# Hongyang-Du/VideoGPA

Measured on AMD Instinct MI355X. Metric: DPO preference-pair steps/sec, CogVideoX-5B 49f@480x720, higher is better.
Workload: dtype bf16; 1 GPU; BASELINE configs[1]: CogVideoX-5B T2V full (42 blocks, D=3072, 48x64 heads), 49f x 480x720 -> paired latents [1,2,13,16,60,90], S=17776 tokens, 42 blocks, LoRA r=64 on to_q/to_k/to_v/to_out.0, 1 pair/GPU/step, optimizer step every step; random-init weights; layers=42, pairs_per_gpu=1, parallelism=dp1

## Files before the change

include/videogpa_hip.h:

```cpp
#ifndef VIDEOGPA_HIP_H
#define VIDEOGPA_HIP_H

#include <stddef.h>
#include <stdint.h>

#ifdef __cplusplus
extern "C" {
#endif

typedef struct ihipStream_t* vgpa_stream_t;

#define VGPA_OK 0
#define VGPA_ERR_INVALID (-1)
#define VGPA_ERR_LAUNCH (-2)
#define VGPA_ERR_WORKSPACE (-3)

size_t vgpa_dpo_loss_workspace_bytes(int64_t B);
int32_t vgpa_dpo_loss_fwd(const void* v_win, const void* v_lose, const void* v_win_ref, const void* v_lose_ref,
                          const void* tgt_win, const void* tgt_lose, int64_t B, int64_t N, int64_t stride_pred,
                          int64_t stride_ref, int64_t stride_tgt, int32_t dtype, float beta, float label_smoothing,
                          int32_t loss_type, int32_t flags, float* out5, float* dlogit, float* errs, void* workspace,
                          size_t ws_bytes, vgpa_stream_t stream);
int32_t vgpa_dpo_loss_bwd(const void* v_win, const void* v_lose, const void* tgt_win, const void* tgt_lose, int64_t B,
                          int64_t N, int64_t stride_pred, int64_t stride_tgt, int64_t stride_grad, int32_t dtype, float beta,
// ... 37 lines not shown
                                int64_t text_len, void* dx, void* dy_q8, float* dy_scale, vgpa_stream_t stream);
int32_t vgpa_gate_residual(const void* x, const void* y, const float* gate_v, const float* gate_t, int64_t mod_stride,
                           int64_t B, int64_t S, int64_t D, int64_t text_len, void* out, vgpa_stream_t stream);
int32_t vgpa_gelu_tanh_fwd(const void* u, int64_t n, void* out, vgpa_stream_t stream);
int32_t vgpa_gelu_tanh_bwd(const void* u, const void* dy, int64_t n, void* du, vgpa_stream_t stream);

int32_t vgpa_qknorm_rope_fwd(const void* q_in, const void* k_in, void* q_out, void* k_out, const int64_t* qin_strides,
                             const int64_t* kin_strides, const int64_t* qout_strides, const int64_t* kout_strides,
                             const float* wq, const float* bq, const float* wk, const float* bk, const float* rope_cos,
                             const float* rope_sin, int64_t text_len, int64_t B, int64_t H, int64_t S, int64_t head_dim,
                             float eps, float q_out_scale, int32_t rope_mode, vgpa_stream_t stream);
int32_t vgpa_qknorm_rope_bwd(const void* dq_out, const void* dk_out, const void* q_in, const void* k_in, void* dq_in,
                             void* dk_in, const int64_t* dqout_strides, const int64_t* dkout_strides,
                             const int64_t* qin_strides, const int64_t* kin_strides, const int64_t* dqin_strides,
                             const int64_t* dkin_strides, const float* wq, const float* wk, const float* rope_cos,
                             const float* rope_sin, int64_t text_len, int64_t B, int64_t H, int64_t S, int64_t head_dim,
                             float eps, int32_t rope_mode, vgpa_stream_t stream);

int32_t vgpa_attn_bwd_delta_res(const void* o, const void* o_res, int32_t res_kind, const void* d_o, const int64_t* o_strides, const int64_t* ores_strides,
                                const int64_t* do_strides, float* delta, int64_t B, int64_t H, int64_t S, int64_t head_dim,
                                vgpa_stream_t stream);
size_t vgpa_attn_bwd_split_workspace_bytes(int64_t B, int64_t H, int64_t S);
int32_t vgpa_attn_bwd_dq_w1(const void* q, const void* k, const void* v, const void* d_o, const float* lse2, const float* delta,
                            void* dq, const int64_t* q_strides, const int64_t* k_strides, const int64_t* v_strides,
                            const int64_t* do_strides, const int64_t* dq_strides, int64_t B, int64_t H, int64_t S, int64_t head_dim,
                            float scale, int32_t split_mode, void* workspace, size_t ws_bytes, vgpa_stream_t stream);
size_t vgpa_attn_fwd_w1_workspace_bytes(int64_t B, int64_t H, int64_t S);
#define VGPA_RES_NONE 0
#define VGPA_RES_BF16 1
#define VGPA_RES_8 2
int32_t vgpa_attn_fwd_w1_res(const void* q, const void* k, const void* v, void* o, void* o_res, int32_t res_kind, float* lse2, const int64_t* q_strides,
                             const int64_t* k_strides, const int64_t* v_strides, const int64_t* o_strides, const int64_t* ores_strides,
                             int64_t B, int64_t H, int64_t S, int64_t head_dim, float scale, int32_t split_mode, void* workspace,
                             size_t ws_bytes, vgpa_stream_t stream);
int32_t vgpa_attn_fwd_online_res(const void* q, const void* k, const void* v, void* o, void* o_res, int32_t res_kind, float* lse2, const int64_t* q_strides,
                                 const int64_t* k_strides, const int64_t* v_strides, const int64_t* o_strides, const int64_t* ores_strides,
                                 int64_t B, int64_t H, int64_t S, int64_t head_dim, float scale, int32_t split_mode, void* workspace,
                                 size_t ws_bytes, vgpa_stream_t stream);
int32_t vgpa_attn_bwd_prep_w1_res(const void* o, const void* o_res, int32_t res_kind, const void* d_o, const float* lse2, const int64_t* o_strides,
                                  const int64_t* ores_strides, const int64_t* do_strides, float* delta, float* stats, int64_t B, int64_t H,
                                  int64_t S, int64_t head_dim, vgpa_stream_t stream);
int32_t vgpa_attn_bwd_dkv_w1(const void* q, const void* k, const void* v, const void* d_o, const float* stats, void* dk, void* dv,
                             const int64_t* q_strides, const int64_t* k_strides, const int64_t* v_strides, const int64_t* do_strides,
                             const int64_t* dk_strides, const int64_t* dv_strides, int64_t B, int64_t H, int64_t S, int64_t head_dim,
                             float scale, int32_t split_mode, void* workspace, size_t ws_bytes, vgpa_stream_t stream);

int32_t vgpa_lora_down(const void* X, int64_t ldx, const void* A, void* T, int64_t ldt, int64_t M, int64_t K, int64_t R,
                       vgpa_stream_t stream);
int32_t vgpa_lora_up_add(void* Y, int64_t ldy, const void* T, int64_t ldt, const void* Bw, int64_t ldb, float s, int64_t M,
                         int64_t N, int64_t rp, int32_t accumulate, vgpa_stream_t stream);
size_t vgpa_lora_grad_workspace_bytes(int64_t M, int64_t P, int64_t Q);
int32_t vgpa_lora_grad_ws(const void* U, int64_t ldu, const void* V, int64_t ldv, float* G, int64_t ldg, float s, int64_t M,
                          int64_t P, int64_t Q, void* workspace, size_t ws_bytes, vgpa_stream_t stream);
int32_t vgpa_lora_ext_refresh(const float* A, const float* B, float s, int64_t r, int64_t K, int64_t Dn, void* a_cat, void* wt_tail, int64_t ld_wt,
                              void* w_tail, int64_t ld_w, void* sbt, vgpa_stream_t stream);

#ifdef VGPA_VARIANTS
int32_t vgpa_gemm_bf16(const void* X, int64_t ldx, const void* W, int64_t ldw, const void* bias, void* C, int64_t ldc, void* aux,
                       int64_t ldaux, int32_t M, int32_t N, int32_t K, int32_t epilogue, vgpa_stream_t stream);
#endif

size_t vgpa_attn128_fwd_workspace_bytes(int64_t B, int64_t H, int64_t Sq);
int32_t vgpa_attn128_fwd(const void* q, const void* k, const void* v, void* o, float* lse2, const int64_t* q_strides, const int64_t* k_strides,
                         const int64_t* v_strides, const int64_t* o_strides, void* o_res8, const int64_t* ores_strides, int64_t B, int64_t H,
                         int64_t Sq, int64_t Skv, float scale, void* workspace, size_t ws_bytes, vgpa_stream_t stream);
size_t vgpa_attn128_fwd_f8_workspace_bytes(int64_t B, int64_t H, int64_t Sq, int64_t Skv);
int32_t vgpa_attn128_fwd_f8(const void* q, const void* k, const void* v, void* o, float* lse2, const int64_t* q_strides, const int64_t* k_strides,
                            const int64_t* v_strides, const int64_t* o_strides, void* o_res8, const int64_t* ores_strides, void* q_deq, void* k_deq,
                            void* v_deq, const int64_t* qd_strides, const int64_t* kd_strides, const int64_t* vd_strides, int64_t B, int64_t H,
                            int64_t Sq, int64_t Skv, float scale, void* workspace, size_t ws_bytes, vgpa_stream_t stream);
size_t vgpa_attn128_bwd_workspace_bytes(int64_t B, int64_t H, int64_t Sq);
int32_t vgpa_attn128_bwd(const void* q, const void* k, const void* v, const void* o, const void* d_o, const float* lse2, void* dq, void* dk,
                         void* dv, const int64_t* q_strides, const int64_t* k_strides, const int64_t* v_strides,
                         const int64_t* o_strides, const int64_t* do_strides, const int64_t* dq_strides, const int64_t* dk_strides,
                         const int64_t* dv_strides, const void* o_res8, const int64_t* ores_strides, int64_t B, int64_t H, int64_t Sq, int64_t Skv,
                         float scale, int32_t dkv_mode, void* workspace, size_t ws_bytes, vgpa_stream_t stream);
int32_t vgpa_attn128_bwd_prescaled(const void* q, const void* k, const void* v, const void* o, const void* d_o, const float* lse2, void* dq, void* dk,
                                   void* dv, const int64_t* q_strides, const int64_t* k_strides, const int64_t* v_strides,
                                   const int64_t* o_strides, const int64_t* do_strides, const int64_t* dq_strides, const int64_t* dk_strides,
                                   const int64_t* dv_strides, const void* o_res8, const int64_t* ores_strides, int64_t B, int64_t H, int64_t Sq, int64_t Skv,
                                   float scale, int32_t dkv_mode, void* workspace, size_t ws_bytes, vgpa_stream_t stream);

int32_t vgpa_wan_ln_mod_fwd(const void* x, int32_t x_dtype, const void* y, const float* gate, float* x_out, const int32_t* gid, const float* ln_w,
                            const float* ln_b, const float* shift, const float* scale, int64_t mod_stride, int64_t rows, int64_t D, float eps,
                            int32_t round_xhat, void* out, int32_t out_dtype, int64_t out_ld, void* q8, float* q8_scale, float* mean, float* rstd,
                            vgpa_stream_t stream);
int32_t vgpa_wan_ln_mod_bwd(const void* dy, int32_t dy_dtype, const void* x, int32_t x_dtype, const float* mean, const float* rstd, const int32_t* gid,
                            const float* ln_w, const float* scale, int64_t mod_stride, int64_t rows, int64_t D, const float* dres, float* dx,
                            const float* gate_prev, void* dy_prev, int64_t ld_dy_prev, vgpa_stream_t stream);
int32_t vgpa_wan_gate_residual(const float* x, const void* y, const int32_t* gid, const float* gate, int64_t mod_stride, int64_t rows, int64_t D, float* out,
                               vgpa_stream_t stream);
int32_t vgpa_wan_gate_bwd(const float* dout, const int32_t* gid, const float* gate, int64_t mod_stride, int64_t rows, int64_t D, void* dy, int64_t ld_dy,
                          vgpa_stream_t stream);
int32_t vgpa_wan_gate_bwd_q8(const float* dout, const int32_t* gid, const float* gate, int64_t mod_stride, int64_t rows, int64_t D, void* q8,
                             float* q8_scale, vgpa_stream_t stream);
int32_t vgpa_wan_rms_rope_fwd(const void* u, int64_t ld_u, const void* w, const float* rope_cos, const float* rope_sin, int64_t L, int64_t head_dim,
                              int64_t rows, int64_t D, float eps, void* out, int64_t ld_out, float* rstd, vgpa_stream_t stream);
int32_t vgpa_wan_rms_rope_bwd(const void* dout, int64_t ld_dout, const void* u, int64_t ld_u, const float* rstd, const void* w, const float* rope_cos,
                              const float* rope_sin, int64_t L, int64_t head_dim, int64_t rows, int64_t D, void* du, int64_t ld_du, vgpa_stream_t stream);

int32_t vgpa_quant_fp8_rows(const void* x, int64_t ldx, void* q, float* scale, int64_t M, int64_t K, vgpa_stream_t stream);
int32_t vgpa_gelu_tanh_fwd_q8(const void* u, int64_t rows, int64_t K, void* q8, float* q8_scale, vgpa_stream_t stream);
int32_t vgpa_gelu_tanh_bwd_q8(const void* u, const void* dy, int64_t rows, int64_t K, void* q8, float* q8_scale, vgpa_stream_t stream);

int32_t vgpa_preprocess_shape(int32_t H, int32_t W, int32_t mode, int32_t* out_h, int32_t* out_w);
size_t vgpa_preprocess_workspace_bytes(int32_t T, int32_t H, int32_t W, int32_t mode);
// ... 159 lines not shown
```

videogpa_amd/_lib.py:

```python
import ctypes
import os

import torch

from ctypes import c_double, c_float, c_int32, c_int64, c_size_t, c_void_p

_HERE = os.path.dirname(os.path.abspath(__file__))
LIB_PATH = os.environ.get("VGPA_LIB") or os.path.join(_HERE, "csrc", "libvgpa_hip.so")

P, I64, I32, F32, F64, SZ = c_void_p, c_int64, c_int32, c_float, c_double, c_size_t

SIGNATURES = {
    "vgpa_dpo_loss_workspace_bytes": (SZ, [I64]),
    "vgpa_dpo_loss_fwd": (I32, [P, P, P, P, P, P, I64, I64, I64, I64, I64, I32, F32, F32, I32, I32, P, P, P, P, SZ, P]),
    "vgpa_dpo_loss_bwd": (I32, [P, P, P, P, I64, I64, I64, I64, I64, I32, F32, I32, P, P, P, P, P]),
    "vgpa_noise_velocity_paired": (I32, [P, P, P, P, P, I64, I64, I32, I32, P, P, P]),
    "vgpa_flow_noise_velocity_paired": (I32, [P, P, P, I64, I64, I32, I32, P, P, P]),
    "vgpa_ln_modulate_fwd": (I32, [P, P, P, P, P, P, P, I64, I64, I64, I64, I64, F32, P, P, P, P]),
    "vgpa_ln_modulate_bwd": (I32, [P, P, P, P, P, P, P, I64, I64, I64, I64, I64, P, P, P]),
    "vgpa_residual_ln_fwd": (I32, [P, P, P, P, I64, P, P, P, P, P, P, I64, I64, I64, I64, I64, F32, P, P, I64, P, P, P]),
    "vgpa_residual_ln_bwd": (I32, [P, P, P, P, P, P, P, I64, P, P, I64, P, I64, I64, I64, I64, P, P, I64, P]),
    "vgpa_residual_ln_fwd_q8": (I32, [P, P, P, P, I64, P, P, P, P, P, P, I64, I64, I64, I64, I64, F32, P, P, P, P, P, P]),
    "vgpa_residual_ln_bwd_q8": (I32, [P, P, P, P, P, P, P, I64, P, P, I64, P, I64, I64, I64, I64, P, P, P, P]),
    "vgpa_gate_residual": (I32, [P, P, P, P, I64, I64, I64, I64, I64, P, P]),
    "vgpa_gelu_tanh_fwd": (I32, [P, I64, P, P]),
    "vgpa_gelu_tanh_bwd": (I32, [P, P, I64, P, P]),
    "vgpa_qknorm_rope_fwd": (I32, [P, P, P, P, P, P, P, P, P, P, P, P, P, P, I64, I64, I64, I64, I64, F32, F32, I32, P]),
    "vgpa_qknorm_rope_bwd": (I32, [P, P, P, P, P, P, P, P, P, P, P, P, P, P, P, P, I64, I64, I64, I64, I64, F32, I32, P]),
    "vgpa_grad_norm_workspace_bytes": (SZ, []),
    "vgpa_grad_norm": (I32, [P, I64, F32, P, P, SZ, P]),
    "vgpa_adamw_step": (I32, [P, P, P, P, I64, F32, F32, F32, F32, F32, I64, F32, F32, P, P]),
    "vgpa_attn_bwd_delta_res": (I32, [P, P, I32, P, P, P, P, P, I64, I64, I64, I64, P]),
    "vgpa_attn_bwd_dq_w1": (I32, [P, P, P, P, P, P, P, P, P, P, P, P, I64, I64, I64, I64, F32, I32, P, SZ, P]),
    "vgpa_attn_fwd_w1_workspace_bytes": (SZ, [I64, I64, I64]),
    "vgpa_attn_bwd_prep_w1_res": (I32, [P, P, I32, P, P, P, P, P, P, P, I64, I64, I64, I64, P]),
    "vgpa_attn_fwd_w1_res": (I32, [P, P, P, P, P, I32, P, P, P, P, P, P, I64, I64, I64, I64, F32, I32, P, SZ, P]),
    "vgpa_attn_fwd_online_res": (I32, [P, P, P, P, P, I32, P, P, P, P, P, P, I64, I64, I64, I64, F32, I32, P, SZ, P]),
    "vgpa_attn_bwd_dkv_w1": (I32, [P, P, P, P, P, P, P, P, P, P, P, P, P, I64, I64, I64, I64, F32, I32, P, SZ, P]),
    "vgpa_attn_bwd_split_workspace_bytes": (SZ, [I64, I64, I64]),
    "vgpa_lora_down": (I32, [P, I64, P, P, I64, I64, I64, I64, P]),
    "vgpa_lora_up_add": (I32, [P, I64, P, I64, P, I64, F32, I64, I64, I64, I32, P]),
    "vgpa_lora_grad_workspace_bytes": (SZ, [I64, I64, I64]),
    "vgpa_lora_grad_ws": (I32, [P, I64, P, I64, P, I64, F32, I64, I64, I64, P, SZ, P]),
    "vgpa_lora_ext_refresh": (I32, [P, P, F32, I64, I64, I64, P, P, I64, P, I64, P, P]),
    "vgpa_attn128_fwd_workspace_bytes": (SZ, [I64, I64, I64]),
    "vgpa_attn128_fwd": (I32, [P, P, P, P, P, P, P, P, P, P, P, I64, I64, I64, I64, F32, P, SZ, P]),
    "vgpa_attn128_fwd_f8_workspace_bytes": (SZ, [I64, I64, I64, I64]),
    "vgpa_attn128_fwd_f8": (I32, [P] * 17 + [I64, I64, I64, I64, F32, P, SZ, P]),
    "vgpa_attn128_bwd_workspace_bytes": (SZ, [I64, I64, I64]),
    "vgpa_attn128_bwd": (I32, [P] * 19 + [I64, I64, I64, I64, F32, I32, P, SZ, P]),
    "vgpa_attn128_bwd_prescaled": (I32, [P] * 19 + [I64, I64, I64, I64, F32, I32, P, SZ, P]),
    "vgpa_wan_ln_mod_fwd": (I32, [P, I32, P, P, P, P, P, P, P, P, I64, I64, I64, F32, I32, P, I32, I64, P, P, P, P, P]),
    "vgpa_wan_ln_mod_bwd": (I32, [P, I32, P, I32, P, P, P, P, P, I64, I64, I64, P, P, P, P, I64, P]),
    "vgpa_wan_gate_residual": (I32, [P, P, P, P, I64, I64, I64, P, P]),
    "vgpa_wan_gate_bwd": (I32, [P, P, P, I64, I64, I64, P, I64, P]),
    "vgpa_wan_gate_bwd_q8": (I32, [P, P, P, I64, I64, I64, P, P, P]),
    "vgpa_wan_rms_rope_fwd": (I32, [P, I64, P, P, P, I64, I64, I64, I64, F32, P, I64, P, P]),
    "vgpa_wan_rms_rope_bwd": (I32, [P, I64, P, I64, P, P, P, P, I64, I64, I64, I64, P, I64, P]),
    "vgpa_quant_fp8_rows": (I32, [P, I64, P, P, I64, I64, P]),
    "vgpa_gelu_tanh_fwd_q8": (I32, [P, I64, I64, P, P, P]),
    "vgpa_gelu_tanh_bwd_q8": (I32, [P, P, I64, I64, P, P, P]),
    "vgpa_preprocess_shape": (I32, [I32, I32, I32, P, P]),
    "vgpa_preprocess_workspace_bytes": (SZ, [I32, I32, I32, I32]),
    "vgpa_preprocess_frames": (I32, [P, I32, I32, I32, I32, P, P, SZ, P]),
    "vgpa_image_resize_workspace_bytes": (SZ, [I32, I32, I32, I32, I32, I32]),
    "vgpa_image_resize": (I32, [P, I32, I32, I32, I32, I32, I32, P, P, SZ, P]),
    "vgpa_image_to_pm1": (I32, [P, I64, I64, I64, I32, P, P]),
    "vgpa_da3_resize_workspace_bytes": (SZ, [I32, I32, I32, I32, I32]),
    "vgpa_da3_resize": (I32, [P, I32, I32, I32, I32, I32, I32, P, P, P, P, P, SZ, P]),
    "vgpa_da3_normalize": (I32, [P, I32, I32, I32, I32, I32, I32, I32, P, P, P, P]),
    "vgpa_sampler_step": (I32, [P, I32, I32, P, P, P, P, I64, I64, I64, I64, I64, I32, F32, F32, F32, F32, F32, F32, F32, P, P, P, I32, P]),
    "vgpa_project_points_workspace_bytes": (SZ, [I64, I64, I64]),
    "vgpa_project_points": (I32, [P, P, P, F32, P, P, P, I32, I64, I64, I64, I64, P, P, P, SZ, P]),
    "vgpa_conf_threshold_workspace_bytes": (SZ, []),
    "vgpa_conf_threshold": (I32, [P, I64, F64, P, P, SZ, P]),
    "vgpa_frame_metric_workspace_bytes": (SZ, []),
    "vgpa_frame_metric": (I32, [P, I32, I32, I32, P, I32, I32, I32, I64, I64, I64, I64, I64, I64, I32, P, P, SZ, P]),
    "vgpa_frame_ssim_workspace_bytes": (SZ, [I64, I64, I64, I64]),
    "vgpa_frame_ssim": (I32, [P, I32, I32, I32, P, I32, I32, I32, I64, I64, I64, I64, I32, P, P, P, SZ, P]),
    "vgpa_frames_to_pm1": (I32, [P, I32, I32, I32, I64, I64, I64, I64, I64, I64, P, P, SZ, P]),
    "vgpa_mvcs_workspace_bytes": (SZ, [I64]),
    "vgpa_mvcs": (I32, [P, P, I32, P, I32, I64, I64, I64, P, P, SZ, P]),
    "vgpa_unproject_depth": (I32, [P, P, P, I32, I64, I64, I64, P, P]),
    "vgpa_pose_decode": (I32, [P, I64, F32, F32, P, P, P]),
    "vgpa_motion_score": (I32, [P, I32, I64, P, P]),
    "vgpa_epipolar_sampson": (I32, [P, P, P, I64, P, P, P]),
    "vgpa_conv3x3_f32": (I32, [P, P, P, P, P, P, I64, I64, I64, I64, I64, I64, I32, P]),
    "vgpa_conv1x1_f32": (I32, [P, P, P, P, I64, I64, I64, P]),
    "vgpa_dpt_tail_f32": (I32, [P, P, P, P, P, P, P, P, P, I64, I64, I64, I64, I64, I64, I32, I32, P]),
    "vgpa_upsample_bilinear_ac_f32": (I32, [P, P, P, P, I64, I64, I64, I64, I64, I64, P]),
    "vgpa_attn_small_f32": (I32, [P, P, P, I64, I64, I64, P, I64, I64, I64, I64, F32, P]),
    "vgpa_dino_embed": (I32, [P, I32, P, I64, P, P, P, P, P, I32, I64, I64, I64, I64, I64, I64, P]),
    "vgpa_stream_ln_f32": (I32, [P, P, P, P, P, P, P, I32, I64, I64, F32, P]),
    "vgpa_lpips_input_f32": (I32, [P, P, I64, I64, I64, F32, F32, F32, F32, F32, F32, I32, P]),
    "vgpa_maxpool2x2_f32": (I32, [P, P, I64, I64, I64, I64, I32, P]),
    "vgpa_lpips_layer_workspace_bytes": (SZ, [I64, I64, I64, I64]),
# ... 89 lines not shown
```

videogpa_amd/csrc/lora.hip:

```cpp
#include "attn_w1.h"

#ifndef LORA_DOWN_DMA
#define LORA_DOWN_DMA 1
#endif
#ifndef LORA_DOWN_DMA_NCB
#define LORA_DOWN_DMA_NCB 2
#endif
#ifndef LORA_DOWN_NS
#define LORA_DOWN_NS 4
#endif
#ifndef LORA_GRAD_WGS
#define LORA_GRAD_WGS 768
#endif

#include <cstdlib>

__device__ __forceinline__ void tile_load_zfill(const bf16_t* base, int64_t ld, int64_t row0, int64_t nrows, int col0, int ncols,
                                                u32x4_t (&r)[2]) {
#pragma unroll
    for (int j = 0; j < 2; ++j) {
        const int c = threadIdx.x + 256 * j;
        const int64_t row = row0 + (c >> 3);
        const int col = col0 + (c & 7) * 8;
        u32x4_t z = {0u, 0u, 0u, 0u};
// ... 260 lines not shown
            tile_load_zfill(U, ldu, mbeg + (int64_t)(t + 1) * 64, mend, p0, P, ur);
            tile_load_zfill(V, ldv, mbeg + (int64_t)(t + 1) * 64, mend, q0, Q, vr);
        }
#pragma unroll
        for (int kc = 0; kc < 4; ++kc) acc = mfma32(frag_tr(ul, 16 * kc, pb * 32, lane), frag_tr(vl, 16 * kc, qb * 32, lane), acc);
        if (t + 1 < nt) {
            tile_store(lds + ((t + 1) & 1) * TILE_ELEMS, ur);
            tile_store(lds + (2 + ((t + 1) & 1)) * TILE_ELEMS, vr);
        }
        __syncthreads();
    }
    const int q = q0 + qb * 32 + (lane & 31);
    if (q < Q) {
        float* slab = part ? part + (int64_t)blockIdx.y * P * Q : nullptr;
#pragma unroll
        for (int r = 0; r < 16; ++r) {
            const int p = p0 + pb * 32 + acc_row(r, hi);
            if (p < P) {
                if (slab) slab[(int64_t)p * Q + q] = acc[r];
                else atomicAdd(&G[(int64_t)p * ldg + q], s * acc[r]);
            }
        }
    }
}

__global__ __launch_bounds__(256) void lora_grad_merge_kernel(const float* __restrict__ part, int nsplit, float* __restrict__ G, int64_t ldg, float s,
                                                                int P, int Q) {
    const int64_t i = (int64_t)blockIdx.x * 256 + threadIdx.x;
    if (i >= (int64_t)P * Q) return;
    float a = 0.f;
    for (int c = 0; c < nsplit; ++c) a += part[(int64_t)c * P * Q + i];
    G[(i / Q) * ldg + (i % Q)] = s * a;
}

__global__ __launch_bounds__(256) void lora_ext_refresh_kernel(const float* __restrict__ A, const float* __restrict__ B, float s, int r, int K, int Dn,
                                                                 bf16_t* __restrict__ a_cat, bf16_t* __restrict__ wt_tail, int64_t ld_wt,
                                                                 bf16_t* __restrict__ w_tail, int64_t ld_w, bf16_t* __restrict__ sbt) {
    const int64_t idx = (int64_t)blockIdx.x * 256 + threadIdx.x;
    const int64_t na = (int64_t)r * K;
    if (idx < na) {
        const int rr = (int)(idx / K), kk = (int)(idx % K);
        const bf16_t a = f32_to_bf16(A[idx]);
        a_cat[idx] = a;
        wt_tail[(int64_t)kk * ld_wt + rr] = a;
    } else if (idx < na + (int64_t)Dn * r) {
        const int64_t e = idx - na;
        const int n = (int)(e / r), rr = (int)(e % r);
        const bf16_t v = f32_to_bf16(bf16_to_f32(f32_to_bf16(B[e])) * s);
        w_tail[(int64_t)n * ld_w + rr] = v;
        sbt[(int64_t)rr * Dn + n] = v;
    }
}

static inline bool a16(const void* p) { return ((uintptr_t)p & 15) == 0; }
static inline bool a8(const void* p) { return ((uintptr_t)p & 7) == 0; }

extern "C" {

int32_t vgpa_lora_down(const void* X, int64_t ldx, const void* A, void* T, int64_t ldt, int64_t M, int64_t K, int64_t R, hipStream_t stream) {
    if (!X || !A || !T || M <= 0 || K <= 0 || K % 64 != 0 || R <= 0 || R > 256 || ldx % 8 || ldt % 8 || ldx < K || ldt < R || !a16(X) || !a16(A) || !a8(T))
        return VGPA_ERR_INVALID;
    if (M > ((int64_t)1 << 31) * 32) return VGPA_ERR_INVALID;
    const int ncb = (int)((R + 31) / 32);
    const dim3 grid((unsigned)((M + 63) / 64));
    constexpr bool dma_off = LORA_DOWN_DMA == 0;
    constexpr int dma_max_ncb = LORA_DOWN_DMA_NCB;
    if (!dma_off && ncb <= dma_max_ncb && (uint64_t)64 * (uint64_t)ldx * 2 + (uint64_t)K * 2 + 1024 < (1ull << 32) && ((uint64_t)R + 8) * (uint64_t)K * 2 + 1024 < (1ull << 32)) {
#define LDD(N, S) VGPA_LAUNCH((lora_down_dma_kernel<N, S>), grid, dim3(256), 0, stream, (const bf16_t*)X, ldx, (const bf16_t*)A, (bf16_t*)T, ldt, M, (int)K, (int)R)
        constexpr int ns = LORA_DOWN_NS;
        switch (ncb * 10 + ns) {
            case 14: LDD(1, 4); break; case 24: LDD(2, 4); break;
            case 13: LDD(1, 3); break; case 23: LDD(2, 3); break;
            case 63: LDD(6, 3); break; case 64: LDD(6, 4); break;
            default: return VGPA_ERR_INVALID;
        }
#undef LDD
        VGPA_CHECK_LAUNCH();
        return VGPA_OK;
    }
    const size_t shmem = (size_t)2 * (64 + 32 * ncb) * PITCH * sizeof(bf16_t);
#define LD(N)                                                                                                                      \
    if (hipFuncSetAttribute((const void*)lora_down_kernel<N>, hipFuncAttributeMaxDynamicSharedMemorySize, (int)shmem) != hipSuccess) \
        return VGPA_ERR_LAUNCH;                                                                                                    \
    VGPA_LAUNCH((lora_down_kernel<N>), grid, dim3(256), shmem, stream, (const bf16_t*)X, ldx, (const bf16_t*)A, (bf16_t*)T, ldt, M, (int)K, (int)R)
    switch (ncb) {
        case 1: LD(1); break; case 2: LD(2); break; case 3: LD(3); break; case 4: LD(4); break;
        case 5: LD(5); break; case 6: LD(6); break; case 7: LD(7); break; case 8: LD(8); break;
        default: return VGPA_ERR_INVALID;
    }
#undef LD
    VGPA_CHECK_LAUNCH();
    return VGPA_OK;
}

int32_t vgpa_lora_up_add(void* Y, int64_t ldy, const void* T, int64_t ldt, const void* Bw, int64_t ldb, float s, int64_t M, int64_t N,
                         int64_t rp, int32_t accumulate, hipStream_t stream) {
    if (!Y || !T || !Bw || M <= 0 || N <= 0 || N % 8 != 0 || ldy % 8 || ldt % 8 || ldb % 8 || !a16(T) || !a16(Bw) || !a16(Y))
        return VGPA_ERR_INVALID;
    if (ldy < N || ldt < rp || ldb < rp) return VGPA_ERR_INVALID;
    const dim3 grid((unsigned)((M + 63) / 64), (unsigned)((N + UP_COLS - 1) / UP_COLS));
#define UP(KS) VGPA_LAUNCH((lora_up_add_kernel<KS>), grid, dim3(256), 0, stream, (bf16_t*)Y, ldy, (const bf16_t*)T, ldt, (const bf16_t*)Bw, ldb, s, M, (int)N, (int)accumulate)
    switch (rp) {
        case 16: UP(1); break; case 32: UP(2); break; case 48: UP(3); break; case 64: UP(4); break;
        case 96: UP(6); break; case 128: UP(8); break; case 192: UP(12); break;
        default: return VGPA_ERR_INVALID;
    }
#undef UP
    VGPA_CHECK_LAUNCH();
    return VGPA_OK;
}

static void lora_grad_plan(int64_t M, int64_t P, int64_t Q, int* n_pt, int* n_qt, int64_t* rows, int64_t* splits) {
    *n_pt = (int)((P + 63) / 64);
    *n_qt = (int)((Q + 63) / 64);
    constexpr int64_t target = LORA_GRAD_WGS;
    int64_t sp = target / ((int64_t)*n_pt * *n_qt);
    if (sp < 1) sp = 1;
    const int64_t max_splits = (M + 255) / 256;
    if (sp > max_splits) sp = max_splits;
    int64_t r = (M + sp - 1) / sp;
    r = (r + 63) / 64 * 64;
    *rows = r;
    *splits = (M + r - 1) / r;
}

size_t vgpa_lora_grad_workspace_bytes(int64_t M, int64_t P, int64_t Q) {
    if (M <= 0 || P <= 0 || Q <= 0) return 0;
    int n_pt, n_qt;
    int64_t rows, splits;
    lora_grad_plan(M, P, Q, &n_pt, &n_qt, &rows, &splits);
    return (size_t)splits * (size_t)P * (size_t)Q * sizeof(float);
}
int32_t vgpa_lora_grad_ws(const void* U, int64_t ldu, const void* V, int64_t ldv, float* G, int64_t ldg, float s, int64_t M, int64_t P,
                          int64_t Q, void* workspace, size_t ws_bytes, hipStream_t stream) {
    if (!U || !V || !G || !workspace || M <= 0 || P <= 0 || Q <= 0 || P % 8 || Q % 8 || ldu % 8 || ldv % 8 || !a16(U) || !a16(V) || !a16(workspace))
        return VGPA_ERR_INVALID;
    if (ldu < P || ldv < Q || ldg < Q || ((uintptr_t)G & 3)) return VGPA_ERR_INVALID;
    int n_pt, n_qt;
    int64_t rows, splits;
    lora_grad_plan(M, P, Q, &n_pt, &n_qt, &rows, &splits);
    if (ws_bytes < (size_t)splits * (size_t)P * (size_t)Q * sizeof(float)) return VGPA_ERR_WORKSPACE;
    VGPA_LAUNCH(lora_grad_kernel, dim3((unsigned)(n_pt * n_qt), (unsigned)splits), dim3(256), 0, stream, (const bf16_t*)U, ldu, (const bf16_t*)V, ldv,
                G, ldg, s, M, (int)P, (int)Q, rows, n_qt, (float*)workspace);
    VGPA_CHECK_LAUNCH();
    VGPA_LAUNCH(lora_grad_merge_kernel, dim3((unsigned)((P * Q + 255) / 256)), dim3(256), 0, stream, (const float*)workspace, (int)splits, G, ldg, s,
                (int)P, (int)Q);
    VGPA_CHECK_LAUNCH();
    return VGPA_OK;
}

int32_t vgpa_lora_ext_refresh(const float* A, const float* B, float s, int64_t r, int64_t K, int64_t Dn, void* a_cat, void* wt_tail, int64_t ld_wt, void* w_tail,
                              int64_t ld_w, void* sbt, hipStream_t stream) {
    if (!A || !B || !a_cat || !wt_tail || !w_tail || !sbt || r <= 0 || K <= 0 || Dn <= 0 || ld_wt < r || ld_w < r) return VGPA_ERR_INVALID;
    const int64_t total = r * K + Dn * r;
    if (total >= ((int64_t)1 << 31)) return VGPA_ERR_INVALID;
    VGPA_LAUNCH(lora_ext_refresh_kernel, dim3((unsigned)((total + 255) / 256)), dim3(256), 0, stream, A, B, s, (int)r, (int)K, (int)Dn, (bf16_t*)a_cat, (bf16_t*)wt_tail,
                ld_wt, (bf16_t*)w_tail, ld_w, (bf16_t*)sbt);
    VGPA_CHECK_LAUNCH();
    return VGPA_OK;
}

}
```

videogpa_amd/ops.py:

```python
import contextlib as _contextlib
import contextvars as _contextvars
import ctypes
import os as _os

import torch

from . import _lib

_DT = {torch.float32: 0, torch.bfloat16: 1}


def _stream():
    return torch.cuda.current_stream().cuda_stream


def _req(t, dtype=None, contiguous=True):
    if not t.is_cuda:
        raise RuntimeError("videogpa_amd ops need GPU tensors (no CPU fallback)")
    if dtype is not None and t.dtype != dtype:
        raise RuntimeError(f"expected {dtype}, got {t.dtype}")
    if contiguous and not t.is_contiguous():
        raise RuntimeError("expected a contiguous tensor")
    return t

# ... 420 lines not shown
    @staticmethod
    def forward(ctx, u):
        _req(u, torch.bfloat16)
        out = _empty_rows(u.shape, u.dtype, u.device, wide=True)
        _timed("gelu_tanh_fwd", 4.0 * u.numel(), lambda: _lib.call("vgpa_gelu_tanh_fwd", u, u.numel(), out, _stream()), "byte")
        ctx.save_for_backward(u)
        return out

    @staticmethod
    def backward(ctx, dy):
        (u,) = ctx.saved_tensors
        dy = dy.contiguous()
        du = _empty_rows(u.shape, u.dtype, u.device, wide=True)
        _timed("gelu_tanh_bwd", 6.0 * u.numel(), lambda: _lib.call("vgpa_gelu_tanh_bwd", u, dy, u.numel(), du, _stream()), "byte")
        return du


def gelu_tanh(u):
    return _GeluTanhFn.apply(u)


def _pad_rank(r):
    rp = 16
    while rp < r:
        rp *= 2
    return rp


def lora_down(x2, a_cat, out=None):
    M, K = x2.shape
    R = a_cat.shape[0]
    t = torch.empty(M, R, dtype=torch.bfloat16, device=x2.device) if out is None else out
    _timed("lora_down_kernel", 2.0 * M * (K + R), lambda: _lib.call("vgpa_lora_down", x2, x2.stride(0), a_cat, t, t.stride(0), M, K, R, _stream()),
           "byte")
    return t


def lora_up_add(y2, t, bw, s, accumulate=True):
    M, N = y2.shape
    _timed("lora_up_add_kernel", (4.0 if accumulate else 2.0) * M * N + 2.0 * M * t.shape[1],
           lambda: _lib.call("vgpa_lora_up_add", y2, y2.stride(0), t, t.stride(0), bw, bw.stride(0), float(s), M, N, t.shape[1],
                             1 if accumulate else 0, _stream()), "byte")


def lora_grad(u, v, s=1.0):
    M, P = u.shape
    Q = v.shape[1]
    g = torch.empty(P, Q, dtype=torch.float32, device=u.device)
    ws_bytes = _lib.query("vgpa_lora_grad_workspace_bytes", M, P, Q)
    ws = torch.empty(ws_bytes, dtype=torch.uint8, device=u.device)
    _timed("lora_grad_kernel", 2.0 * M * (P + Q), lambda: _lib.call("vgpa_lora_grad_ws", u, u.stride(0), v, v.stride(0), g, Q, float(s), M, P, Q,
                                                                     ws, ws_bytes, _stream()), "byte")
    return g


TUNED_GEMM_FILE = _os.path.join(_os.path.dirname(_os.path.abspath(__file__)), "tuned", "tunableop_gfx950.csv")
_TUNED_GEMMS = None


def use_tuned_gemms(enabled=True, path=None):
    global _TUNED_GEMMS
    import torch.cuda.tunable as tn
    if _os.environ.get("PYTORCH_TUNABLEOP_ENABLED") is not None:
        gpu = torch.cuda.is_available()
        _TUNED_GEMMS = {"enabled": tn.is_enabled() if gpu else False, "file": tn.get_filename() if gpu else None, "entries": None,
                        "note": "PYTORCH_TUNABLEOP_* set by the caller: left as is"}
        return _TUNED_GEMMS
    path = path or TUNED_GEMM_FILE
    if not torch.cuda.is_available():
        _TUNED_GEMMS = {"enabled": False, "file": None, "entries": 0}
        return _TUNED_GEMMS
    if not enabled or not _os.path.isfile(path):
        if _TUNED_GEMMS is not None and _TUNED_GEMMS.get("enabled"):
            tn.enable(False)
        _TUNED_GEMMS = {"enabled": False, "file": None, "entries": 0}
        return _TUNED_GEMMS
    if _TUNED_GEMMS is not None and _TUNED_GEMMS.get("enabled") and _TUNED_GEMMS.get("file") == path:
        return _TUNED_GEMMS
    with open(path) as f:
        entries = sum(1 for ln in f if ln.startswith(("Gemm", "ScaledGemm")))
    tn.enable(True)
    tn.tuning_enable(False)
    tn.record_untuned_enable(False)
    tn.set_filename(path, False)
    _TUNED_GEMMS = {"enabled": True, "file": path, "entries": entries}
    return _TUNED_GEMMS


def tuned_gemms_state():
    return _TUNED_GEMMS


_WT_CACHE = True


def _transposed(W):
    if not _WT_CACHE:
        return None
    c = getattr(W, "_vgpa_wt", None)
    if c is None or c[0] != W._version or c[1].device != W.device or c[1].dtype != W.dtype:
        c = (W._version, W.detach().t().contiguous())
        W._vgpa_wt = c
    return c[1]


GEMM_SPLIT_OVERRIDE = None
# ... 329 lines not shown
        _, s1v, _, s1t, mstride = _mod_ptrs(mod2)
        _timed("residual_ln_bwd", 10.0 * rows * D,
               lambda: _lib.call("vgpa_residual_ln_bwd", dh, x1, mean1, rstd1, ln_w, s1v, s1t, mstride, gates1[:, 0], gates1[:, 1], gates1.stride(0),
                                 dx1, B, S, D, ctx.text_len, dx, da, D + dyp, _stream()), "byte")
        return (dx, da) + (None,) * 17


def ffn_tail_fp8(x, a, gates1, ln_w, ln_b, mod2, W1, b1, W2, b2, gates2, nxt_w, nxt_b, nxt_mod=None, nxt_eps=1e-5, text_len=0, eps=1e-5, n_pad=0, dy_pad=0):
    if W1.requires_grad or W2.requires_grad or (b1 is not None and b1.requires_grad) or (b2 is not None and b2.requires_grad):
        raise RuntimeError("videogpa_amd: the fp8 path is for frozen projections only")
    if W1.shape[0] > 16384:
        raise RuntimeError(f"ffn_tail_fp8: the GELU -> e4m3 kernels hold one feed-forward row per workgroup, inner <= 16384; got {W1.shape[0]}")
    return _FfnTailFp8Fn.apply(x, a, gates1, ln_w, ln_b, mod2, W1, b1, W2, b2, gates2, nxt_w, nxt_b, nxt_mod, nxt_eps, int(text_len), eps, int(n_pad),
                               int(dy_pad))


class _LinearLoraExtFn(torch.autograd.Function):

    @staticmethod
    def forward(ctx, x, bias, ext, enabled, scalings, x_recompute, *AB):
        K, R, N = ext.K, ext.R, ext.N
        x2 = x.reshape(-1, K)
        M = x2.shape[0]
        x_ext = _padded_base(x2, K + R)
        if x_ext is None:
            x_ext = torch.zeros(M, K + R, dtype=x.dtype, device=x.device) if not enabled else torch.empty(M, K + R, dtype=x.dtype, device=x.device)
            x_ext[:, :K].copy_(x2)
        xv, tv = x_ext[:, :K], x_ext[:, K:]
        if enabled:
            lora_down(xv, ext.A_cat, out=tv)
        ctx.rows_per_call = current_gemm_rows()
        y = _gemm(x_ext, ext.W_ext, bias, ext=True, split=ctx.rows_per_call)
        if x_recompute is not None and enabled:
            fn, srcs = x_recompute
            ctx.save_for_backward(tv.contiguous(), *srcs)
            ctx.x_fn = fn
        else:
            ctx.save_for_backward(x_ext)
            ctx.x_fn = None
        ctx.ext, ctx.enabled, ctx.xshape, ctx.scalings = ext, enabled, x.shape, scalings
        return y.view(*x.shape[:-1], N)

    @staticmethod
    def backward(ctx, dy):
        ext, enabled = ctx.ext, ctx.enabled
        saved, *srcs = ctx.saved_tensors
        K, R, N, Dn, rp, r, act = ext.K, ext.R, ext.N, ext.Dn, ext.rp, ext.r, ext.act
        dy2 = dy.reshape(-1, N)
        M = dy2.shape[0]
        dy_ext = _padded_base(dy2, N + R) if dy2.stride(1) == 1 else None
        if dy_ext is None:
            dy_ext = torch.zeros(M, N + R, dtype=dy.dtype, device=dy.device) if not enabled else torch.empty(M, N + R, dtype=dy.dtype, device=dy.device)
            dy_ext[:, :N].copy_(dy2)
        if enabled:
            for j, i in enumerate(act):
                lora_down(dy_ext[:, i * Dn:(i + 1) * Dn], ext.sBt[j], out=dy_ext[:, N + j * rp:N + (j + 1) * rp])
        dx = _gemm(dy_ext, ext.Wt_ext, ext=True, split=ctx.rows_per_call)
        out_grads = [None] * len(ctx.needs_input_grad[6:])
        if enabled:
            if ctx.x_fn is not None:
                t_all, xh = saved, ctx.x_fn(*srcs).reshape(M, K)
            else:
                t_all, xh = saved[:, K:], saved[:, :K]
            for j, i in enumerate(act):
                out_grads[2 * i + 1] = lora_grad(dy_ext[:, i * Dn:(i + 1) * Dn], t_all[:, j * rp:(j + 1) * rp], ctx.scalings[j])[:, :r]
            dA = lora_grad(dy_ext[:, N:], xh)
            for j, i in enumerate(act):
                out_grads[2 * i] = dA[j * rp:j * rp + r]
        return (dx.view(ctx.xshape), None, None, None, None, None, *out_grads)


def linear_lora_ext(x, W, bias, ext, loras, enabled=True, x_recompute=None):
    if W.requires_grad or (bias is not None and bias.requires_grad):
        raise RuntimeError("videogpa_amd: base weights are frozen on this path (LoRA-only training, as in the reference)")
    ext.refresh(W, len(loras), loras)
    flat = []
    for l in loras:
        flat += [None, None] if l is None else [l[0], l[1]]
    return _LinearLoraExtFn.apply(x, bias, ext, bool(enabled), tuple(float(loras[i][2]) for i in ext.act), x_recompute, *flat)


def linear_lora(x, W, bias, loras, ext=None):
    if all(l is None for l in loras):
        return frozen_linear(x, W, bias)
    if ext is None:
        ext = getattr(W, "_vgpa_lora_ext", None)
        if ext is None:
            ext = LoraExt()
            W._vgpa_lora_ext = ext
    return linear_lora_ext(x, W, bias, ext, loras, True)


def _bhs_strides(t):
    assert t.stride(3) == 1
    return _i64x3(t.stride(0), t.stride(1), t.stride(2))


LOG2E = 1.4426950408889634
ATTN_SPLIT_MODE = -1
def precise_delta_default():
    v = _os.environ.get("VGPA_PRECISE_DELTA", "int8").lower()
    if v in ("0", "off", "none", "false"):
        return None
    if v in ("1", "int8", "res8", "true"):
        return "int8"
    if v == "bf16":
        return "bf16"
    raise ValueError(f"VGPA_PRECISE_DELTA={v!r}: expected 0 | off | int8 | bf16")


def _res_kind(o_res):
    if o_res is None:
        return 0
    if o_res.dtype == torch.bfloat16:
        return 1
    if o_res.dtype == torch.uint8:
        return 2
# ... 1139 lines not shown
```

Before: 0.4365 pair-steps/s.

## Fuse LoRA backward down-projection and B-gradient into one streaming kernel

Adds a fused HIP kernel that reads each dY column slice once and computes both the LoRA down-projection (dY·sB^T into the extended dy buffer) and the B-weight gradient (dY^T·T) for all active adapters. Partial sums go to a workspace split across column strips and row ranges, and a merge kernel reduces them. This replaces the per-adapter lora_down and lora_grad launches, so dY is no longer streamed twice per adapter. In exchange it adds fp32 workspace traffic, an extra merge launch, and a per-call workspace allocation.

After: 0.4353 pair-steps/s. No clear change (-0.3%).

```diff
diff --git a/include/videogpa_hip.h b/include/videogpa_hip.h
--- a/include/videogpa_hip.h
+++ b/include/videogpa_hip.h
@@ -113,6 +113,9 @@
 size_t vgpa_lora_grad_workspace_bytes(int64_t M, int64_t P, int64_t Q);
 int32_t vgpa_lora_grad_ws(const void* U, int64_t ldu, const void* V, int64_t ldv, float* G, int64_t ldg, float s, int64_t M,
                           int64_t P, int64_t Q, void* workspace, size_t ws_bytes, vgpa_stream_t stream);
+size_t vgpa_lora_bwd_workspace_bytes(int64_t M, int64_t Dn, int64_t rp, int64_t n_act);
+int32_t vgpa_lora_bwd(void* dy_ext, int64_t ld, const void* sBt, const void* T_all, int64_t ldt, float* dB, const int32_t* slices, const float* scalings,
+                      int64_t M, int64_t N, int64_t Dn, int64_t rp, int64_t n_act, void* workspace, size_t ws_bytes, vgpa_stream_t stream);
 int32_t vgpa_lora_ext_refresh(const float* A, const float* B, float s, int64_t r, int64_t K, int64_t Dn, void* a_cat, void* wt_tail, int64_t ld_wt,
                               void* w_tail, int64_t ld_w, void* sbt, vgpa_stream_t stream);
 
diff --git a/videogpa_amd/_lib.py b/videogpa_amd/_lib.py
--- a/videogpa_amd/_lib.py
+++ b/videogpa_amd/_lib.py
@@ -42,6 +42,8 @@
     "vgpa_lora_up_add": (I32, [P, I64, P, I64, P, I64, F32, I64, I64, I64, I32, P]),
     "vgpa_lora_grad_workspace_bytes": (SZ, [I64, I64, I64]),
     "vgpa_lora_grad_ws": (I32, [P, I64, P, I64, P, I64, F32, I64, I64, I64, P, SZ, P]),
+    "vgpa_lora_bwd_workspace_bytes": (SZ, [I64, I64, I64, I64]),
+    "vgpa_lora_bwd": (I32, [P, I64, P, P, I64, P, P, P, I64, I64, I64, I64, I64, P, SZ, P]),
     "vgpa_lora_ext_refresh": (I32, [P, P, F32, I64, I64, I64, P, P, I64, P, I64, P, P]),
     "vgpa_attn128_fwd_workspace_bytes": (SZ, [I64, I64, I64]),
     "vgpa_attn128_fwd": (I32, [P, P, P, P, P, P, P, P, P, P, P, I64, I64, I64, I64, F32, P, SZ, P]),
diff --git a/videogpa_amd/csrc/lora.hip b/videogpa_amd/csrc/lora.hip
--- a/videogpa_amd/csrc/lora.hip
+++ b/videogpa_amd/csrc/lora.hip
@@ -336,6 +336,156 @@
     }
 }
 
+#include "lora_bwd_plan.h"
+
+struct LoraBwdSlices {
+    int32_t col0[LORA_BWD_MAX_ACT];
+    float scale[LORA_BWD_MAX_ACT];
+};
+
+template <int NCH, int NS>
+__global__ __launch_bounds__(256) void lora_bwd_kernel(const bf16_t* __restrict__ dY, int64_t ld, const bf16_t* __restrict__ sBt, const bf16_t* __restrict__ T,
+                                                         int64_t ldt, LoraBwdSlices sl, int64_t M, int Dn, int rp, int64_t rows_per_range, int64_t Mp,
+                                                         float* __restrict__ dtp, float* __restrict__ dbp) {
+    constexpr uint32_t STAGE = 16384u;
+    constexpr uint32_t TBASE = (uint32_t)NS * STAGE;
+    constexpr int PW = 4;
+    __shared__ __attribute__((aligned(1024))) uint8_t lds[NS * (STAGE + 8192)];
+    const int lane = threadIdx.x & 63, hi = lane >> 5;
+    const int wave = __builtin_amdgcn_readfirstlane((int)threadIdx.x >> 6);
+    const int rb = wave & 1, cg = wave >> 1;
+    const int strip = blockIdx.x, range = blockIdx.y, j = blockIdx.z;
+    const int nstrips = gridDim.x, nranges = gridDim.y;
+    const int col0 = strip * NCH * 64;
+    const int left = (Dn - col0) / 64;
+    const int nch = left < NCH ? left : NCH;
+    const int64_t mbeg = (int64_t)range * rows_per_range;
+    const int64_t rows = (M - mbeg) < rows_per_range ? (M - mbeg) : rows_per_range;
+    const int ntiles = (int)((rows + 63) / 64);
+
+    const W1Rsrc xrs = w1_rsrc(dY + mbeg * ld + sl.col0[j] + col0, (uint32_t)(((rows - 1) * ld + nch * 64) * 2));
+    const W1Rsrc ars = w1_rsrc(sBt + (int64_t)j * rp * Dn + col0, (uint32_t)(((int64_t)(rp - 1) * Dn + nch * 64) * 2));
+    const W1Rsrc trs = w1_rsrc(T + mbeg * ldt + j * rp, (uint32_t)(((rows - 1) * ldt + rp) * 2));
+    uint32_t xo[2], ao[2], to[2];
+#pragma unroll
+    for (int i = 0; i < 2; ++i) {
+        const uint32_t row = 8u * (uint32_t)(wave * 2 + i) + (uint32_t)(lane >> 3);
+        const uint32_t c = (((uint32_t)(lane & 7) ^ w1_swz(row)) * 8u);
+        xo[i] = (uint32_t)((row * (uint64_t)ld + c) * 2u);
+        ao[i] = (row * (uint32_t)Dn + c) * 2u;
+        to[i] = (uint32_t)((row * (uint64_t)ldt + c) * 2u);
+    }
+    const uint32_t lds0 = (uint32_t)(uintptr_t)(__attribute__((address_space(3))) uint8_t*)lds;
+    const uint32_t wdst = __builtin_amdgcn_readfirstlane(lds0 + (uint32_t)wave * 2048u);
+    int ic = 0, islot = 0, itslot = 0;
+    uint32_t xrun = 0u, arun = 0u, trun = 0u;
+    const uint32_t xrow = (uint32_t)(64 * ld * 2) - (uint32_t)(nch * 128), trow = (uint32_t)(64 * ldt * 2);
+    auto issue = [&]() {
+        const uint32_t so = wdst + (uint32_t)islot * STAGE;
+#pragma unroll
+        for (int i = 0; i < 2; ++i) w1_dma(so + 1024u * i, xrs, xo[i] + xrun, 0u);
+#pragma unroll
+        for (int i = 0; i < 2; ++i) w1_dma(so + 8192u + 1024u * i, ars, ao[i] + arun, 0u);
+        if (ic == 0) {
+            const uint32_t td = wdst + TBASE + (uint32_t)itslot * 8192u;
+#pragma unroll
+            for (int i = 0; i < 2; ++i) w1_dma(td + 1024u * i, trs, to[i] + trun, 0u);
+        }
+        islot = islot + 1 == NS ? 0 : islot + 1;
+        ++ic;
+        xrun += 128u;
+        arun += 128u;
+        if (ic == nch) {
+            ic = 0;
+            xrun += xrow;
+            arun = 0u;
+            trun += trow;
+            itslot = itslot + 1 == NS ? 0 : itslot + 1;
+        }
+    };
+    f32x16_t acc_t, acc_b[NCH];
+#pragma unroll
+    for (int i = 0; i < 16; ++i) acc_t[i] = 0.f;
+#pragma unroll
+    for (int c = 0; c < NCH; ++c)
+#pragma unroll
+        for (int i = 0; i < 16; ++i) acc_b[c][i] = 0.f;
+    const W1Lane la = w1_lane_offsets(lane);
+#pragma unroll
+    for (int t = 0; t < NS - 1; ++t) issue();
+    int slot = 0, tslot = 0;
+    float* dt_out = dtp + (((int64_t)j * nstrips + strip) * rp + cg * 32 + 4 * hi) * Mp + mbeg + rb * 32 + (lane & 31);
+    for (int tile = 0; tile < ntiles; ++tile) {
+        const uint32_t tb = TBASE + (uint32_t)tslot * 8192u;
+#pragma unroll
+        for (int c = 0; c < NCH; ++c) {
+            if (c < nch) {
+                lora_wait_vm<PW * (NS - 2)>();
+                __builtin_amdgcn_s_barrier();
+                issue();
+                const uint32_t xb = (uint32_t)slot * STAGE, ab = xb + 8192u;
+#pragma unroll
+                for (int ks = 0; ks < 4; ++ks)
+                    acc_t = mfma32(w1_frag_row(lds, ab, la, cg, ks), w1_frag_row(lds, xb, la, rb, ks), acc_t);
+#pragma unroll
+                for (int kc = 0; kc < 4; ++kc)
+                    acc_b[c] = mfma32(w1_frag_tr(lds, xb, la, kc >> 1, kc & 1, rb), w1_frag_tr(lds, tb, la, kc >> 1, kc & 1, cg), acc_b[c]);
+                slot = slot + 1 == NS ? 0 : slot + 1;
+            }
+        }
+#pragma unroll
+        for (int r = 0; r < 16; ++r) {
+            if (cg * 32 + acc_row(r, hi) < rp) dt_out[(int64_t)((r & 3) + 8 * (r >> 2)) * Mp] = acc_t[r];
+            acc_t[r] = 0.f;
+        }
+        dt_out += 64;
+        tslot = tslot + 1 == NS ? 0 : tslot + 1;
+    }
+    lora_wait_vm<0>();
+    const int q = cg * 32 + (lane & 31);
+    if (q < rp) {
+        float* slab = dbp + (((int64_t)j * nranges + range) * Dn + col0 + rb * 32) * rp + q;
+#pragma unroll
+        for (int c = 0; c < NCH; ++c) {
+            if (c < nch) {
+#pragma unroll
+                for (int r = 0; r < 16; ++r) slab[(int64_t)(c * 64 + acc_row(r, hi)) * rp] = acc_b[c][r];
+            }
+        }
+    }
+}
+
+__global__ __launch_bounds__(256) void lora_bwd_merge_kernel(const float* __restrict__ dtp, const float* __restrict__ dbp, bf16_t* __restrict__ dY, int64_t ld,
+                                                               float* __restrict__ dB, LoraBwdSlices sl, int64_t M, int64_t Mp, int N, int Dn, int rp, int n_act,
+                                                               int nstrips, int nranges, int64_t nb_dt) {
+    if ((int64_t)blockIdx.x < nb_dt) {
+        const int64_t idx = (int64_t)blockIdx.x * 256 + threadIdx.x;
+        const int ng = rp / 8;
+        const int64_t m = idx % Mp;
+        const int64_t jg = idx / Mp;
+        const int g = (int)(jg % ng), j = (int)(jg / ng);
+        if (j >= n_act || m >= M) return;
+        float o[8];
+#pragma unroll
+        for (int i = 0; i < 8; ++i) o[i] = 0.f;
+        for (int s = 0; s < nstrips; ++s) {
+            const float* p = dtp + (((int64_t)j * nstrips + s) * rp + g * 8) * Mp + m;
+#pragma unroll
+            for (int i = 0; i < 8; ++i) o[i] += p[(int64_t)i * Mp];
+        }
+        *reinterpret_cast<u32x4_t*>(dY + m * ld + N + j * rp + g * 8) = pack8(o);
+    } else {
+        const int64_t per = (int64_t)Dn * rp;
+        const int64_t idx = ((int64_t)blockIdx.x - nb_dt) * 256 + threadIdx.x;
+        if (idx >= per * n_act) return;
+        const int j = (int)(idx / per);
+        const int64_t e = idx % per;
+        float a = 0.f;
+        for (int c = 0; c < nranges; ++c) a += dbp[((int64_t)j * nranges + c) * per + e];
+        dB[idx] = sl.scale[j] * a;
+    }
+}
+
 static inline bool a16(const void* p) { return ((uintptr_t)p & 15) == 0; }
 static inline bool a8(const void* p) { return ((uintptr_t)p & 7) == 0; }
 
@@ -433,6 +583,33 @@
     return VGPA_OK;
 }
 
+size_t vgpa_lora_bwd_workspace_bytes(int64_t M, int64_t Dn, int64_t rp, int64_t n_act) {
+    LoraBwdPlan p;
+    if (!lora_bwd_plan(M, Dn, rp, n_act, &p)) return 0;
+    return p.dt_bytes + p.db_bytes;
+}
+int32_t vgpa_lora_bwd(void* dy_ext, int64_t ld, const void* sBt, const void* T_all, int64_t ldt, float* dB, const int32_t* slices, const float* scalings, int64_t M,
+                      int64_t N, int64_t Dn, int64_t rp, int64_t n_act, void* workspace, size_t ws_bytes, hipStream_t stream) {
+    LoraBwdPlan p;
+    const int32_t rc = lora_bwd_check(dy_ext, ld, sBt, T_all, ldt, dB, slices, scalings, M, N, Dn, rp, n_act, workspace, ws_bytes, &p);
+    if (rc != 0) return rc;
+    LoraBwdSlices sl = {};
+    for (int64_t j = 0; j < n_act; ++j) {
+        sl.col0[j] = (int32_t)(slices[j] * Dn);
+        sl.scale[j] = scalings[j];
+    }
+    float* dtp = (float*)workspace;
+    float* dbp = (float*)((uint8_t*)workspace + p.dt_bytes);
+    VGPA_LAUNCH((lora_bwd_kernel<LORA_BWD_NCH, LORA_BWD_NS>), dim3((unsigned)p.nstrips, (unsigned)p.nranges, (unsigned)n_act), dim3(256), 0, stream,
+                (const bf16_t*)dy_ext, ld, (const bf16_t*)sBt, (const bf16_t*)T_all, ldt, sl, M, (int)Dn, (int)rp, p.rows, p.Mp, dtp, dbp);
+    VGPA_CHECK_LAUNCH();
+    const int64_t nb_dt = (n_act * (rp / 8) * p.Mp + 255) / 256, nb_db = (n_act * Dn * rp + 255) / 256;
+    VGPA_LAUNCH(lora_bwd_merge_kernel, dim3((unsigned)(nb_dt + nb_db)), dim3(256), 0, stream, (const float*)dtp, (const float*)dbp, (bf16_t*)dy_ext, ld, dB, sl, M,
+                p.Mp, (int)N, (int)Dn, (int)rp, (int)n_act, (int)p.nstrips, (int)p.nranges, nb_dt);
+    VGPA_CHECK_LAUNCH();
+    return VGPA_OK;
+}
+
 int32_t vgpa_lora_ext_refresh(const float* A, const float* B, float s, int64_t r, int64_t K, int64_t Dn, void* a_cat, void* wt_tail, int64_t ld_wt, void* w_tail,
                               int64_t ld_w, void* sbt, hipStream_t stream) {
     if (!A || !B || !a_cat || !wt_tail || !w_tail || !sbt || r <= 0 || K <= 0 || Dn <= 0 || ld_wt < r || ld_w < r) return VGPA_ERR_INVALID;
diff --git a/videogpa_amd/csrc/lora_bwd_plan.h b/videogpa_amd/csrc/lora_bwd_plan.h
--- /dev/null
+++ b/videogpa_amd/csrc/lora_bwd_plan.h
@@ -0,0 +1,57 @@
+#pragma once
+#include <cstddef>
+#include <cstdint>
+
+#ifndef LORA_BWD_NCH
+#define LORA_BWD_NCH 16
+#endif
+#ifndef LORA_BWD_NS
+#define LORA_BWD_NS 6
+#endif
+#ifndef LORA_BWD_WGS
+#define LORA_BWD_WGS 256
+#endif
+#define LORA_BWD_MAX_ACT 8
+
+struct LoraBwdPlan {
+    int64_t nstrips, rows, nranges, Mp;
+    size_t dt_bytes, db_bytes;
+};
+
+static inline bool lora_bwd_plan(int64_t M, int64_t Dn, int64_t rp, int64_t n_act, LoraBwdPlan* p) {
+    if (M <= 0 || Dn <= 0 || Dn % 64 != 0 || (rp != 16 && rp != 32 && rp != 64) || n_act <= 0 || n_act > LORA_BWD_MAX_ACT) return false;
+    if (M > ((int64_t)1 << 31) || Dn > ((int64_t)1 << 24)) return false;
+    const int64_t cs = (int64_t)LORA_BWD_NCH * 64;
+    p->nstrips = (Dn + cs - 1) / cs;
+    int64_t sp = (int64_t)LORA_BWD_WGS / (p->nstrips * n_act);
+    if (sp < 1) sp = 1;
+    const int64_t max_splits = (M + 255) / 256;
+    if (sp > max_splits) sp = max_splits;
+    int64_t r = (M + sp - 1) / sp;
+    r = (r + 63) / 64 * 64;
+    p->rows = r;
+    p->nranges = (M + r - 1) / r;
+    p->Mp = (M + 63) / 64 * 64;
+    p->dt_bytes = (size_t)n_act * (size_t)p->nstrips * (size_t)rp * (size_t)p->Mp * sizeof(float);
+    p->db_bytes = (size_t)n_act * (size_t)p->nranges * (size_t)Dn * (size_t)rp * sizeof(float);
+    return true;
+}
+
+static inline int32_t lora_bwd_check(const void* dy_ext, int64_t ld, const void* sBt, const void* T_all, int64_t ldt, const void* dB, const int32_t* slices,
+                                     const float* scalings, int64_t M, int64_t N, int64_t Dn, int64_t rp, int64_t n_act, const void* workspace, size_t ws_bytes,
+                                     LoraBwdPlan* p) {
+    auto al = [](const void* q, uintptr_t a) { return ((uintptr_t)q & (a - 1)) == 0; };
+    if (!dy_ext || !sBt || !T_all || !dB || !slices || !scalings || !workspace) return -1;
+    if (N <= 0 || N % 8 != 0 || N >= ((int64_t)1 << 31) || ld % 8 != 0 || ldt % 8 != 0) return -1;
+    if (!lora_bwd_plan(M, Dn, rp, n_act, p)) return -1;
+    if (ld < N + n_act * rp || ldt < n_act * rp) return -1;
+    if (!al(dy_ext, 16) || !al(sBt, 16) || !al(T_all, 16) || !al(dB, 4) || !al(workspace, 16)) return -1;
+    for (int64_t j = 0; j < n_act; ++j)
+        if (slices[j] < 0 || ((int64_t)slices[j] + 1) * Dn > N) return -1;
+    const int64_t span = p->rows + 64 * (LORA_BWD_NS + 2);
+    const int64_t wide = ld > ldt ? ld : ldt;
+    if ((uint64_t)span * (uint64_t)wide * 2 + ((uint64_t)1 << 20) >= ((uint64_t)1 << 32)) return -1;
+    if ((uint64_t)(rp + 64) * (uint64_t)Dn * 2 + ((uint64_t)1 << 20) >= ((uint64_t)1 << 32)) return -1;
+    if (ws_bytes < p->dt_bytes + p->db_bytes) return -3;
+    return 0;
+}
diff --git a/videogpa_amd/ops.py b/videogpa_amd/ops.py
--- a/videogpa_amd/ops.py
+++ b/videogpa_amd/ops.py
@@ -496,6 +496,27 @@
     _timed("lora_grad_kernel", 2.0 * M * (P + Q), lambda: _lib.call("vgpa_lora_grad_ws", u, u.stride(0), v, v.stride(0), g, Q, float(s), M, P, Q,
                                                                      ws, ws_bytes, _stream()), "byte")
     return g
+
+
+LORA_BWD_FUSED = True
+
+
+def lora_bwd_workspace_bytes(M, Dn, rp, n_act):
+    return _lib.query("vgpa_lora_bwd_workspace_bytes", M, Dn, rp, n_act)
+
+
+def lora_bwd(dy_ext, N, Dn, rp, slices, sbt, t_all, scalings):
+    M, n_act = dy_ext.shape[0], len(slices)
+    ws_bytes = lora_bwd_workspace_bytes(M, Dn, rp, n_act)
+    if ws_bytes == 0:
+        raise RuntimeError(f"lora_bwd: no kernel for M {M}, Dn {Dn}, rp {rp}, {n_act} adapters")
+    ws = torch.empty(ws_bytes, dtype=torch.uint8, device=dy_ext.device)
+    dB = torch.empty(n_act, Dn, rp, dtype=torch.float32, device=dy_ext.device)
+    sl = (ctypes.c_int32 * n_act)(*[int(i) for i in slices])
+    sc = (ctypes.c_float * n_act)(*[float(v) for v in scalings])
+    _timed("lora_bwd_kernel", 2.0 * M * (N + n_act * rp) + ws_bytes,
+           lambda: _lib.call("vgpa_lora_bwd", dy_ext, dy_ext.stride(0), sbt, t_all, t_all.stride(0), dB, sl, sc, M, N, Dn, rp, n_act, ws, ws_bytes, _stream()), "byte")
+    return dB
 
 
 TUNED_GEMM_FILE = _os.path.join(_os.path.dirname(_os.path.abspath(__file__)), "tuned", "tunableop_gfx950.csv")
@@ -931,17 +952,23 @@
         if dy_ext is None:
             dy_ext = torch.zeros(M, N + R, dtype=dy.dtype, device=dy.device) if not enabled else torch.empty(M, N + R, dtype=dy.dtype, device=dy.device)
             dy_ext[:, :N].copy_(dy2)
+        dB_all = None
         if enabled:
-            for j, i in enumerate(act):
-                lora_down(dy_ext[:, i * Dn:(i + 1) * Dn], ext.sBt[j], out=dy_ext[:, N + j * rp:N + (j + 1) * rp])
+            t_all = saved if ctx.x_fn is not None else saved[:, K:]
+            if (LORA_BWD_FUSED and dy_ext.dtype == torch.bfloat16 and dy_ext.is_cuda and K % 8 == 0 and N % 8 == 0 and t_all.data_ptr() % 16 == 0
+                    and lora_bwd_workspace_bytes(M, Dn, rp, len(act)) > 0):
+                dB_all = lora_bwd(dy_ext, N, Dn, rp, act, ext.sBt, t_all, ctx.scalings)
+            else:
+                for j, i in enumerate(act):
+                    lora_down(dy_ext[:, i * Dn:(i + 1) * Dn], ext.sBt[j], out=dy_ext[:, N + j * rp:N + (j + 1) * rp])
         dx = _gemm(dy_ext, ext.Wt_ext, ext=True, split=ctx.rows_per_call)
         out_grads = [None] * len(ctx.needs_input_grad[6:])
         if enabled:
-            if ctx.x_fn is not None:
-                t_all, xh = saved, ctx.x_fn(*srcs).reshape(M, K)
-            else:
-                t_all, xh = saved[:, K:], saved[:, :K]
+            xh = ctx.x_fn(*srcs).reshape(M, K) if ctx.x_fn is not None else saved[:, :K]
             for j, i in enumerate(act):
+                if dB_all is not None:
+                    out_grads[2 * i + 1] = dB_all[j, :, :r]
+                    continue
                 out_grads[2 * i + 1] = lora_grad(dy_ext[:, i * Dn:(i + 1) * Dn], t_all[:, j * rp:(j + 1) * rp], ctx.scalings[j])[:, :r]
             dA = lora_grad(dy_ext[:, N:], xh)
             for j, i in enumerate(act):
```
